# facebookresearch/goliath

Measured on NVIDIA B200. Metric: rendered megapixels/sec (fwd+bwd) RGCA head 300k Gaussians, higher is better.
Workload: dtype f32

## Files before the change

### goliath_b200/csrc/splat_bin_tiles.cu

```cuda
#include <stdlib.h>
#include <string.h>

#include "common.cuh"
#include "splat_record.cuh"

extern "C" int gb_tile_order(int num_tiles, const int32_t* tile_bins, int32_t* order, void* stream);
extern "C" int gb_tile_schedule(int num_tiles, const int32_t* tile_bins, int32_t* sched, void* stream);
GB_API int gb_bin_tiles_pack_ev(int G, const float* xys, const float* depths, const int32_t* radii, const float* conics,
                                const float* colors3, const float* opacity, const float* compensation, int img_h,
                                int img_w, int block_width, int64_t cap, int32_t* tile_bins, int32_t* tile_order,
                                int tile_sched, int32_t* gids_sorted, float* records, int32_t* n_out, int32_t* overflow,
                                void* workspace, void* colors_ready, void* stream);

namespace {

constexpr int kRankBlock = 256;
constexpr int kRadix = 256;
constexpr int kRankPasses = 4;
constexpr int kScatItems = 2;
constexpr int kSortThreads = 512;
constexpr int kCopyBatch = 2;
constexpr int kMaxBitmapBytes = 192 * 1024;
constexpr int kMaxSmemTiles = 20 * 1024;

inline int rank_items(int G) { return G <= 2048 * 192 ? 8 : 16; }

__device__ __forceinline__ int block_exclusive_scan(int v, int* s_warp, int& total) {
  const int lane = threadIdx.x & 31, warp = threadIdx.x >> 5;
  int inc = v;
#pragma unroll
  for (int o = 1; o < 32; o <<= 1) {
    int t = __shfl_up_sync(0xffffffffu, inc, o);
    if (lane >= o) inc += t;
  }
  if (lane == 31) s_warp[warp] = inc;
  __syncthreads();
  if (warp == 0) {
    int w = (lane < (int)(blockDim.x >> 5)) ? s_warp[lane] : 0;
    int winc = w;
#pragma unroll
    for (int o = 1; o < 32; o <<= 1) {
      int t = __shfl_up_sync(0xffffffffu, winc, o);
      if (lane >= o) winc += t;
    }
    s_warp[lane] = winc - w;
    if (lane == 31) s_warp[32] = winc;
  }
  __syncthreads();
  total = s_warp[32];
  const int r = s_warp[warp] + inc - v;
  __syncthreads();
  return r;
}

__device__ __forceinline__ void tile_bbox(float cx, float cy, float radius, int tbx, int tby, int bw, int& x0,
                                          int& y0, int& x1, int& y1) {
  const float fb = (float)bw;
  const float tcx = __fdiv_rn(cx, fb), tcy = __fdiv_rn(cy, fb), tr = __fdiv_rn(radius, fb);
  x0 = min(max(0, __float2int_rz(__fsub_rn(tcx, tr))), tbx);
  x1 = min(max(0, __float2int_rz(__fadd_rn(__fadd_rn(tcx, tr), 1.f))), tbx);
  y0 = min(max(0, __float2int_rz(__fsub_rn(tcy, tr))), tby);
  y1 = min(max(0, __float2int_rz(__fadd_rn(__fadd_rn(tcy, tr), 1.f))), tby);
}

constexpr int kGaussBlock = 1024;
template <int kTileKeys, bool kRank>
__global__ void __launch_bounds__(kGaussBlock) depth_keys_kernel(int G, const float2* __restrict__ xys,
                                                                 const float* __restrict__ depths,
                                                                 const int* __restrict__ radii, int tbx, int tby,
                                                                 int block_width, int smem_tiles,
                                                                 unsigned* __restrict__ keys,
                                                                 unsigned* __restrict__ hist0 ,
                                                                 int* __restrict__ tile_counts,
                                                                 unsigned* __restrict__ key_bits ) {
  constexpr int kItems = kTileKeys / kGaussBlock;
  extern __shared__ int s_cnt[];
  __shared__ unsigned s_hist[kRadix];
  __shared__ unsigned s_or, s_orc, s_max, s_maxc;
  if (threadIdx.x == 0) s_or = s_orc = s_max = s_maxc = 0u;
  if (threadIdx.x < kRadix) s_hist[threadIdx.x] = 0;
  for (int t = threadIdx.x; t < smem_tiles; t += kGaussBlock) s_cnt[t] = 0;
  const int base = blockIdx.x * kTileKeys;
  unsigned k[kItems];
  int r[kItems];
  float2 c[kItems];
#pragma unroll
  for (int j = 0; j < kItems; ++j) {
    const int i = base + j * kGaussBlock + threadIdx.x;
    const bool in = i < G;
    k[j] = in ? __float_as_uint(depths[i]) : 0u;
    r[j] = in ? radii[i] : 0;
    c[j] = in ? xys[i] : make_float2(0.f, 0.f);
  }
  {
    unsigned o = 0u, oc = 0u, mx = 0u, mxc = 0u;
#pragma unroll
    for (int j = 0; j < kItems; ++j)
      if (r[j] > 0) { o |= k[j]; oc |= ~k[j]; mx = max(mx, k[j]); mxc = max(mxc, ~k[j]); }
    o = __reduce_or_sync(0xffffffffu, o);
    oc = __reduce_or_sync(0xffffffffu, oc);
    mx = __reduce_max_sync(0xffffffffu, mx);
    mxc = __reduce_max_sync(0xffffffffu, mxc);
    __syncthreads();
    if ((threadIdx.x & 31) == 0 && (o | oc)) {
      atomicOr(&s_or, o); atomicOr(&s_orc, oc); atomicMax(&s_max, mx); atomicMax(&s_maxc, mxc);
    }
  }
  __syncthreads();
#pragma unroll
  for (int j = 0; j < kItems; ++j) {
    const int i = base + j * kGaussBlock + threadIdx.x;
    if (i >= G) continue;
    if (kRank) {
      keys[i] = k[j];
      atomicAdd(&s_hist[k[j] & 0xffu], 1u);
    }
    if (r[j] > 0) {
      int x0, y0, x1, y1;
      tile_bbox(c[j].x, c[j].y, (float)r[j], tbx, tby, block_width, x0, y0, x1, y1);
      for (int ty = y0; ty < y1; ++ty)
        for (int tx = x0; tx < x1; ++tx) {
          if (smem_tiles) atomicAdd(&s_cnt[ty * tbx + tx], 1);
          else atomicAdd(&tile_counts[ty * tbx + tx], 1);
        }
    }
  }
  __syncthreads();
  if (threadIdx.x == 0 && (s_or | s_orc)) {
    atomicOr(key_bits, s_or); atomicOr(key_bits + 1, s_orc);
    atomicMax(key_bits + 4, s_max); atomicMax(key_bits + 5, s_maxc);
  }
  if (kRank && threadIdx.x < kRadix) hist0[(size_t)blockIdx.x * kRadix + threadIdx.x] = s_hist[threadIdx.x];
  for (int t = threadIdx.x; t < smem_tiles; t += kGaussBlock) {
    const int cnt = s_cnt[t];
    if (cnt) atomicAdd(&tile_counts[t], cnt);
  }
}

template <int kItems>
__global__ void __launch_bounds__(kRankBlock) rank_scatter_kernel(
    int n, const unsigned* __restrict__ keys_in, const int* __restrict__ vals_in ,
    unsigned* __restrict__ keys_out , int* __restrict__ vals_out, int shift, int ctas,
    const unsigned* __restrict__ hist_cur ,
    unsigned* __restrict__ hist_next ,
    int* __restrict__ rank_of ) {
  constexpr int kWarps = kRankBlock / 32;
  constexpr int kTile = kRankBlock * kItems;
  __shared__ unsigned s_whist[kWarps][kRadix];
  __shared__ int s_scan[33];
  const int lane = threadIdx.x & 31, warp = threadIdx.x >> 5;

  const int warp_base = blockIdx.x * kTile + warp * (32 * kItems);
  unsigned k[kItems];
  int v[kItems];
#pragma unroll
  for (int j = 0; j < kItems; ++j) {
    const int i = warp_base + j * 32 + lane;
    k[j] = (i < n) ? keys_in[i] : 0xffffffffu;
    v[j] = (i < n) ? (vals_in ? vals_in[i] : i) : 0;
  }

  __shared__ uint4 s_part[2][4][kRadix / 4];
  {
    const int g = threadIdx.x >> 6, c4 = threadIdx.x & 63;
    const uint4* tab = reinterpret_cast<const uint4*>(hist_cur);
    uint4 tot = make_uint4(0u, 0u, 0u, 0u), bef = make_uint4(0u, 0u, 0u, 0u);
#pragma unroll 8
    for (int b = g; b < ctas; b += 4) {
      const uint4 h = tab[(size_t)b * (kRadix / 4) + c4];
      tot.x += h.x; tot.y += h.y; tot.z += h.z; tot.w += h.w;
      if (b < (int)blockIdx.x) { bef.x += h.x; bef.y += h.y; bef.z += h.z; bef.w += h.w; }
    }
    s_part[0][g][c4] = tot;
    s_part[1][g][c4] = bef;
  }
  __syncthreads();
  unsigned before = 0, total = 0;
  {
    const unsigned* pt = reinterpret_cast<const unsigned*>(&s_part[0][0][0]);
    const unsigned* pb = reinterpret_cast<const unsigned*>(&s_part[1][0][0]);
#pragma unroll
    for (int g = 0; g < 4; ++g) {
      total += pt[g * kRadix + threadIdx.x];
      before += pb[g * kRadix + threadIdx.x];
    }
  }
  const bool copy_only = __syncthreads_or(total == (unsigned)n) != 0;

  if (copy_only) {
#pragma unroll
    for (int j = 0; j < kItems; ++j) {
      const int i = warp_base + j * 32 + lane;
      if (i < n) {
        if (keys_out) keys_out[i] = k[j];
        vals_out[i] = v[j];
        if (hist_next) atomicAdd(&hist_next[(size_t)blockIdx.x * kRadix + ((k[j] >> (shift + 8)) & 0xffu)], 1u);
        if (rank_of) rank_of[v[j]] = i;
      }
    }
    return;
  }
  int unused;
  const unsigned digit_base = (unsigned)block_exclusive_scan((int)total, s_scan, unused);
  const unsigned my_base = digit_base + before;

  for (int d = lane; d < kRadix; d += 32) s_whist[warp][d] = 0;
  __syncwarp();
  unsigned rank[kItems];
#pragma unroll
  for (int j = 0; j < kItems; ++j) {
    const int i = warp_base + j * 32 + lane;
    const bool valid = i < n;
    const unsigned dgt = (k[j] >> shift) & 0xffu;
    const unsigned peers = __match_any_sync(0xffffffffu, valid ? dgt : 0x100u);
    const unsigned lower = peers & ((1u << lane) - 1u);
    unsigned prev = 0;
    if (valid) prev = s_whist[warp][dgt];
    __syncwarp();
    rank[j] = prev + __popc(lower);
    if (valid && lower == 0u) s_whist[warp][dgt] = prev + __popc(peers);
    __syncwarp();
  }
  __syncthreads();
  {
    const int d = threadIdx.x;
    unsigned run = my_base;
#pragma unroll
    for (int w = 0; w < kWarps; ++w) {
      const unsigned c = s_whist[w][d];
      s_whist[w][d] = run;
      run += c;
    }
  }
  __syncthreads();
#pragma unroll
  for (int j = 0; j < kItems; ++j) {
    const int i = warp_base + j * 32 + lane;
    if (i < n) {
      const unsigned dgt = (k[j] >> shift) & 0xffu;
      const unsigned dst = s_whist[warp][dgt] + rank[j];
      if (keys_out) keys_out[dst] = k[j];
      vals_out[dst] = v[j];
      if (hist_next) atomicAdd(&hist_next[(size_t)(dst / kTile) * kRadix + ((k[j] >> (shift + 8)) & 0xffu)], 1u);
      if (rank_of) rank_of[v[j]] = (int)dst;
    }
  }
}


__device__ __forceinline__ void grid_barrier(unsigned* counter, unsigned& target) {
  __syncthreads();
  if (threadIdx.x == 0) {
    target += gridDim.x;
    __threadfence();
    atomicAdd(counter, 1u);
    unsigned seen;
    do {
      asm volatile("ld.acquire.gpu.global.u32 %0, [%1];" : "=r"(seen) : "l"(counter) : "memory");
    } while (seen < target);
    __threadfence();
  }
  __syncthreads();
}

template <int kItems>
__global__ void __launch_bounds__(kRankBlock) rank_sort_coop_kernel(
    int n, int tiles, unsigned* keys_a, unsigned* keys_b, int* vals_a, int* vals_b, unsigned* hist ,
    const unsigned* key_bits, unsigned* barrier , int* __restrict__ rank_to_gid, int* __restrict__ rank_of) {
  constexpr int kWarps = kRankBlock / 32;
  constexpr int kTile = kRankBlock * kItems;
  __shared__ unsigned s_whist[kWarps][kRadix];
  __shared__ int s_scan[33];
  __shared__ uint4 s_part[2][4][kRadix / 4];
  const int lane = threadIdx.x & 31, warp = threadIdx.x >> 5;
  if (key_bits[7] && !key_bits[6]) return;
  const unsigned diff = key_bits[0] & key_bits[1];
  const int bits = diff ? 32 - __clz(diff) : 0;
  const int passes = (bits + 7) >> 3;
  unsigned bar_target = 0;
  const size_t hs = (size_t)tiles * kRadix;

  if (passes == 0) {
    for (int i = blockIdx.x * kRankBlock + threadIdx.x; i < n; i += gridDim.x * kRankBlock) {
      rank_to_gid[i] = i;
      rank_of[i] = i;
    }
    return;
  }
  auto warp_ranks = [&](const unsigned (&k)[kItems], int warp_base, int shift, unsigned (&rank)[kItems]) {
    for (int d = lane; d < kRadix; d += 32) s_whist[warp][d] = 0;
    __syncwarp();
#pragma unroll
    for (int j = 0; j < kItems; ++j) {
      const int i = warp_base + j * 32 + lane;
      const bool valid = i < n;
      const unsigned dgt = (k[j] >> shift) & 0xffu;
      const unsigned peers = __match_any_sync(0xffffffffu, valid ? dgt : 0x100u);
      const unsigned lower = peers & ((1u << lane) - 1u);
      unsigned prev = 0;
      if (valid) prev = s_whist[warp][dgt];
      __syncwarp();
      rank[j] = prev + __popc(lower);
      if (valid && lower == 0u) s_whist[warp][dgt] = prev + __popc(peers);
      __syncwarp();
    }
  };
  for (int p = 0; p < passes; ++p) {
    const bool last = (p == passes - 1);
    const int shift = 8 * p;
    const unsigned* kin = (p & 1) ? keys_b : keys_a;
    unsigned* kout = (p & 1) ? keys_a : keys_b;
    const int* vin = (p == 0) ? nullptr : ((p & 1) ? vals_b : vals_a);
    int* vout = last ? rank_to_gid : ((p & 1) ? vals_a : vals_b);
    unsigned* hist_cur = hist + (size_t)p * hs;
    if (p > 0) {
      for (int tile = blockIdx.x; tile < tiles; tile += gridDim.x) {
        const int warp_base = tile * kTile + warp * (32 * kItems);
        unsigned k[kItems], rank[kItems];
#pragma unroll
        for (int j = 0; j < kItems; ++j) {
          const int i = warp_base + j * 32 + lane;
          k[j] = (i < n) ? __ldcg(kin + i) : 0xffffffffu;
        }
        warp_ranks(k, warp_base, shift, rank);
        __syncthreads();
        {
          unsigned c = 0;
#pragma unroll
          for (int w = 0; w < kWarps; ++w) c += s_whist[w][threadIdx.x];
          hist_cur[(size_t)tile * kRadix + threadIdx.x] = c;
        }
        __syncthreads();
      }
      grid_barrier(barrier, bar_target);
    }
    for (int tile = blockIdx.x; tile < tiles; tile += gridDim.x) {
      const int warp_base = tile * kTile + warp * (32 * kItems);
      unsigned k[kItems];
      int v[kItems];
#pragma unroll
      for (int j = 0; j < kItems; ++j) {
        const int i = warp_base + j * 32 + lane;
        k[j] = (i < n) ? __ldcg(kin + i) : 0xffffffffu;
        v[j] = (i < n) ? (vin ? __ldcg(vin + i) : i) : 0;
      }
      {
        const int g = threadIdx.x >> 6, c4 = threadIdx.x & 63;
        const uint4* tab = reinterpret_cast<const uint4*>(hist_cur);
        uint4 tot = make_uint4(0u, 0u, 0u, 0u), bef = make_uint4(0u, 0u, 0u, 0u);
#pragma unroll 8
        for (int b = g; b < tiles; b += 4) {
          const uint4 h = __ldcg(tab + (size_t)b * (kRadix / 4) + c4);
          tot.x += h.x; tot.y += h.y; tot.z += h.z; tot.w += h.w;
          if (b < tile) { bef.x += h.x; bef.y += h.y; bef.z += h.z; bef.w += h.w; }
        }
        s_part[0][g][c4] = tot;
        s_part[1][g][c4] = bef;
      }
      __syncthreads();
      unsigned before = 0, total = 0;
      {
        const unsigned* pt = reinterpret_cast<const unsigned*>(&s_part[0][0][0]);
        const unsigned* pb = reinterpret_cast<const unsigned*>(&s_part[1][0][0]);
#pragma unroll
        for (int g = 0; g < 4; ++g) {
          total += pt[g * kRadix + threadIdx.x];
          before += pb[g * kRadix + threadIdx.x];
        }
      }
      int unused;
      const unsigned digit_base = (unsigned)block_exclusive_scan((int)total, s_scan, unused);
      const unsigned my_base = digit_base + before;
      unsigned rank[kItems];
      warp_ranks(k, warp_base, shift, rank);
      __syncthreads();
      {
        const int d = threadIdx.x;
        unsigned run = my_base;
#pragma unroll
        for (int w = 0; w < kWarps; ++w) {
          const unsigned c = s_whist[w][d];
          s_whist[w][d] = run;
          run += c;
        }
      }
      __syncthreads();
#pragma unroll
      for (int j = 0; j < kItems; ++j) {
        const int i = warp_base + j * 32 + lane;
        if (i < n) {
          const unsigned dgt = (k[j] >> shift) & 0xffu;
          const unsigned dst = s_whist[warp][dgt] + rank[j];
          if (!last) kout[dst] = k[j];
          else rank_of[v[j]] = (int)dst;
          vout[dst] = v[j];
        }
      }
      __syncthreads();
    }
    if (!last) grid_barrier(barrier, bar_target);
  }
}

constexpr int kBuckets = 2048;
constexpr int kBucketCap = 2048;
constexpr int kBucketThreads = 128;

__device__ __forceinline__ int bucket_of(unsigned key, unsigned kmin, unsigned long long range) {
  return (int)(((unsigned long long)(key - kmin) * (unsigned long long)kBuckets) / range);
}

template <int kTileKeys>
__global__ void __launch_bounds__(kGaussBlock) rank_bucket_count_kernel(int G, const unsigned* __restrict__ keys,
                                                                        const int* __restrict__ radii,
                                                                        const unsigned* __restrict__ key_bits,
                                                                        int* __restrict__ bcount) {
  constexpr int kItems = kTileKeys / kGaussBlock;
  __shared__ int s_cnt[kBuckets];
  for (int t = threadIdx.x; t < kBuckets; t += kGaussBlock) s_cnt[t] = 0;
  const unsigned kmax = key_bits[4], kmin = ~key_bits[5];
  const unsigned long long range = (unsigned long long)(kmax - kmin) + 1ull;
  __syncthreads();
  const int base = blockIdx.x * kTileKeys;
#pragma unroll
  for (int j = 0; j < kItems; ++j) {
    const int i = base + j * kGaussBlock + threadIdx.x;
    if (i < G && radii[i] > 0) atomicAdd(&s_cnt[bucket_of(keys[i], kmin, range)], 1);
  }
  __syncthreads();
  for (int t = threadIdx.x; t < kBuckets; t += kGaussBlock) {
    const int c = s_cnt[t];
    if (c) atomicAdd(&bcount[t], c);
  }
}

__global__ void __launch_bounds__(1024) rank_bucket_scan_kernel(const int* __restrict__ bcount, int* __restrict__ boffset,
                                                                int* __restrict__ bcursor, unsigned* __restrict__ flags) {
  __shared__ int s_warp[33];
  __shared__ int s_max;
  if (threadIdx.x == 0) s_max = 0;
  __syncthreads();
  int carry = 0;
  for (int base = 0; base < kBuckets; base += 1024) {
    const int i = base + threadIdx.x;
    const int v = bcount[i];
    int total;
    const int ex = block_exclusive_scan(v, s_warp, total);
    boffset[i] = carry + ex;
    bcursor[i] = 0;
    atomicMax(&s_max, v);
    carry += total;
  }
  __syncthreads();
  if (threadIdx.x == 0) flags[6] = (s_max > kBucketCap) ? 1u : 0u;
}

template <int kTileKeys>
__global__ void __launch_bounds__(kGaussBlock) rank_bucket_scatter_kernel(int G, const unsigned* __restrict__ keys,
                                                                          const int* __restrict__ radii,
                                                                          const unsigned* __restrict__ key_bits,
                                                                          const int* __restrict__ boffset,
                                                                          int* __restrict__ bcursor,
                                                                          unsigned* __restrict__ pair_keys,
                                                                          int* __restrict__ pair_ids) {
  constexpr int kItems = kTileKeys / kGaussBlock;
  __shared__ int s_cnt[kBuckets];
  __shared__ int s_base[kBuckets];
  if (key_bits[6]) return;
  for (int t = threadIdx.x; t < kBuckets; t += kGaussBlock) s_cnt[t] = 0;
  const unsigned kmax = key_bits[4], kmin = ~key_bits[5];
  const unsigned long long range = (unsigned long long)(kmax - kmin) + 1ull;
  __syncthreads();
  const int base = blockIdx.x * kTileKeys;
  unsigned k[kItems];
  int b[kItems];
#pragma unroll
  for (int j = 0; j < kItems; ++j) {
    const int i = base + j * kGaussBlock + threadIdx.x;
    b[j] = -1;
    if (i < G && radii[i] > 0) {
      k[j] = keys[i];
      b[j] = bucket_of(k[j], kmin, range);
      atomicAdd(&s_cnt[b[j]], 1);
    }
  }
  __syncthreads();
  for (int t = threadIdx.x; t < kBuckets; t += kGaussBlock) {
    const int c = s_cnt[t];
    s_base[t] = c ? boffset[t] + atomicAdd(&bcursor[t], c) : 0;
    s_cnt[t] = 0;
  }
  __syncthreads();
#pragma unroll
  for (int j = 0; j < kItems; ++j) {
    if (b[j] < 0) continue;
    const int pos = s_base[b[j]] + atomicAdd(&s_cnt[b[j]], 1);
    pair_keys[pos] = k[j];
    pair_ids[pos] = base + j * kGaussBlock + threadIdx.x;
  }
}

__global__ void __launch_bounds__(kBucketThreads) rank_bucket_sort_kernel(const int* __restrict__ bcount,
                                                                          const int* __restrict__ boffset,
                                                                          const unsigned* __restrict__ key_bits,
                                                                          const unsigned* __restrict__ pair_keys,
                                                                          const int* __restrict__ pair_ids,
                                                                          int* __restrict__ rank_to_gid, int* __restrict__ rank_of) {
  __shared__ unsigned s_k[kBucketCap];
  __shared__ int s_id[kBucketCap];
  if (key_bits[6]) return;
  const int n = bcount[blockIdx.x], off = boffset[blockIdx.x];
  if (n <= 0) return;
  for (int i = threadIdx.x; i < n; i += kBucketThreads) {
    s_k[i] = pair_keys[off + i];
    s_id[i] = pair_ids[off + i];
  }
  __syncthreads();
  for (int i = threadIdx.x; i < n; i += kBucketThreads) {
    const unsigned ki = s_k[i];
    const int idi = s_id[i];
    int r = 0;
    for (int j = 0; j < n; ++j) {
      const unsigned kj = s_k[j];
      r += (kj < ki || (kj == ki && s_id[j] < idi)) ? 1 : 0;
    }
    rank_to_gid[off + r] = idi;
    rank_of[idi] = off + r;
  }
}

__global__ void __launch_bounds__(1024) tile_scan_kernel(int T, long long cap, const int* __restrict__ counts,
                                                         int2* __restrict__ tile_bins, int* __restrict__ cursor,
                                                         int* __restrict__ n_out, int* __restrict__ overflow) {
  __shared__ int s_warp[33];
  int carry = 0;
  for (int base = 0; base < T; base += blockDim.x) {
    const int i = base + threadIdx.x;
    const int v = (i < T) ? counts[i] : 0;
    int total;
    const int ex = block_exclusive_scan(v, s_warp, total);
    if (i < T) {
      const int s = carry + ex;
      cursor[i] = s;
      const int cs = (int)min((long long)s, cap), ce = (int)min((long long)s + v, cap);
      tile_bins[i] = (ce > cs) ? make_int2(cs, ce) : make_int2(0, 0);
    }
    carry += total;
  }
  if (threadIdx.x == 0) {
    if (n_out) *n_out = carry;
    if (overflow && (long long)carry > cap) *overflow = 1;
  }
}

template <bool kById>
__global__ void __launch_bounds__(kGaussBlock) tile_scatter_kernel(
    int G, const float2* __restrict__ xys, const int* __restrict__ radii, const int* __restrict__ rank_of,
    const float* __restrict__ conics, const float* __restrict__ colors3, const float* __restrict__ depths,
    const float* __restrict__ opacity, const float* __restrict__ comp, int tbx, int tby, int block_width,
    long long cap, int smem_tiles, int* __restrict__ cursor, int* __restrict__ tile_ranks, int* __restrict__ slot_ids,
    float4* __restrict__ rec_by_rank) {
  extern __shared__ int s_cnt[];
  int* s_base = s_cnt + smem_tiles;
  for (int t = threadIdx.x; t < smem_tiles; t += kGaussBlock) s_cnt[t] = 0;
  const int base = blockIdx.x * (kGaussBlock * kScatItems);
  int rk[kScatItems], r[kScatItems];
  float2 c[kScatItems];
#pragma unroll
  for (int j = 0; j < kScatItems; ++j) {
    const int i = base + j * kGaussBlock + threadIdx.x;
    const bool in = i < G;
    r[j] = in ? radii[i] : 0;
    c[j] = in ? xys[i] : make_float2(0.f, 0.f);
    if (kById) rk[j] = in ? __float_as_int(depths[i]) : 0;
    else rk[j] = in ? rank_of[i] : 0;
  }
  __syncthreads();
  unsigned bx[kScatItems], by[kScatItems];
#pragma unroll
  for (int j = 0; j < kScatItems; ++j) {
    const int i = base + j * kGaussBlock + threadIdx.x;
    bx[j] = by[j] = 0u;
    if (r[j] <= 0) continue;
    int x0, y0, x1, y1;
    tile_bbox(c[j].x, c[j].y, (float)r[j], tbx, tby, block_width, x0, y0, x1, y1);
    bx[j] = (unsigned)x0 | ((unsigned)x1 << 16);
    by[j] = (unsigned)y0 | ((unsigned)y1 << 16);
    gb::pack_record_fused(i, xys, conics, colors3, depths, opacity, comp, rec_by_rank + 3 * (size_t)(kById ? i : rk[j]));
    for (int ty = y0; ty < y1; ++ty)
      for (int tx = x0; tx < x1; ++tx) {
        if (smem_tiles) {
          atomicAdd(&s_cnt[ty * tbx + tx], 1);
        } else {
          const int pos = atomicAdd(&cursor[ty * tbx + tx], 1);
          if ((long long)pos < cap) {
            tile_ranks[pos] = rk[j];
            if (kById) slot_ids[pos] = i;
          }
        }
      }
  }
  if (!smem_tiles) return;
  __syncthreads();
  for (int t = threadIdx.x; t < smem_tiles; t += kGaussBlock) {
    const int cnt = s_cnt[t];
    s_base[t] = cnt ? atomicAdd(&cursor[t], cnt) : 0;
    s_cnt[t] = 0;
  }
  __syncthreads();
#pragma unroll
  for (int j = 0; j < kScatItems; ++j) {
    const int x0 = bx[j] & 0xffffu, x1 = bx[j] >> 16, y0 = by[j] & 0xffffu, y1 = by[j] >> 16;
    for (int ty = y0; ty < y1; ++ty)
      for (int tx = x0; tx < x1; ++tx) {
        const int t = ty * tbx + tx;
        const int pos = s_base[t] + atomicAdd(&s_cnt[t], 1);
        if ((long long)pos < cap) {
          tile_ranks[pos] = rk[j];
          if (kById) slot_ids[pos] = base + j * kGaussBlock + threadIdx.x;
        }
      }
  }
}

__global__ void __launch_bounds__(kSortThreads, 3) tile_sort_pack_kernel(
    int words , int chunk , const int* __restrict__ order,
    const int2* __restrict__ tile_bins, const int* __restrict__ tile_ranks, const int* __restrict__ rank_to_gid,
    const float4* __restrict__ rec_by_rank, int* __restrict__ gids_sorted, float4* __restrict__ rec) {
  extern __shared__ unsigned s_bits[];
  __shared__ int s_warp[33];
  const int tile = order ? order[blockIdx.x] : (int)blockIdx.x;
  const int2 range = tile_bins[tile];
  const int n = range.y - range.x;
  if (n <= 0) return;
  for (int w = threadIdx.x; w < words; w += kSortThreads) s_bits[w] = 0u;
  __syncthreads();
  for (int i0 = threadIdx.x; i0 < n; i0 += 4 * kSortThreads) {
    int r[4];
#pragma unroll
    for (int u = 0; u < 4; ++u) {
      const int i = i0 + u * kSortThreads;
      r[u] = (i < n) ? tile_ranks[range.x + i] : -1;
    }
#pragma unroll
    for (int u = 0; u < 4; ++u)
      if (r[u] >= 0) atomicOr(&s_bits[r[u] >> 5], 1u << (r[u] & 31));
  }
  __syncthreads();
  const int w0 = threadIdx.x * chunk, w1 = min(words, w0 + chunk);
  int cnt = 0;
  for (int w = w0; w < w1; ++w) cnt += __popc(s_bits[w]);
  int total;
  int pos = range.x + block_exclusive_scan(cnt, s_warp, total);
  for (int w = w0; w < w1; ++w) {
    unsigned m = s_bits[w];
    while (m) {
      const int b = __ffs(m) - 1;
      m &= m - 1;
      gids_sorted[pos++] = w * 32 + b;
    }
  }
  __syncthreads();
  for (int i0 = threadIdx.x; i0 < n; i0 += kCopyBatch * kSortThreads) {
    int r[kCopyBatch], g[kCopyBatch];
    float4 q[kCopyBatch][3];
#pragma unroll
    for (int u = 0; u < kCopyBatch; ++u) {
      const int i = i0 + u * kSortThreads;
      r[u] = (i < n) ? __ldcg(gids_sorted + (size_t)range.x + i) : -1;
    }
#pragma unroll
    for (int u = 0; u < kCopyBatch; ++u) {
      if (r[u] < 0) continue;
      g[u] = rank_to_gid[r[u]];
      const float4* src = rec_by_rank + 3 * (size_t)r[u];
      q[u][0] = gb::ld_nc_f4(src);
      q[u][1] = gb::ld_nc_f4(src + 1);
      q[u][2] = gb::ld_nc_f4(src + 2);
    }
#pragma unroll
    for (int u = 0; u < kCopyBatch; ++u) {
      if (r[u] < 0) continue;
      const size_t idx = (size_t)range.x + i0 + u * kSortThreads;
      gids_sorted[idx] = g[u];
      rec[3 * idx + 0] = q[u][0];
      rec[3 * idx + 1] = q[u][1];
      rec[3 * idx + 2] = q[u][2];
    }
  }
}

__global__ void __launch_bounds__(kSortThreads, 3) tile_sort_kernel(int words, int chunk, const int* __restrict__ order,
                                                                    const int2* __restrict__ tile_bins,
                                                                    int* __restrict__ tile_ranks) {
  extern __shared__ unsigned s_bits[];
  __shared__ int s_warp[33];
  const int tile = order ? order[blockIdx.x] : (int)blockIdx.x;
  const int2 range = tile_bins[tile];
  const int n = range.y - range.x;
  if (n <= 0) return;
  for (int w = threadIdx.x; w < words; w += kSortThreads) s_bits[w] = 0u;
  __syncthreads();
  for (int i0 = threadIdx.x; i0 < n; i0 += 4 * kSortThreads) {
    int r[4];
#pragma unroll
    for (int u = 0; u < 4; ++u) {
      const int i = i0 + u * kSortThreads;
      r[u] = (i < n) ? tile_ranks[range.x + i] : -1;
    }
#pragma unroll
    for (int u = 0; u < 4; ++u)
      if (r[u] >= 0) atomicOr(&s_bits[r[u] >> 5], 1u << (r[u] & 31));
  }
  __syncthreads();
  const int w0 = threadIdx.x * chunk, w1 = min(words, w0 + chunk);
  int cnt = 0;
  for (int w = w0; w < w1; ++w) cnt += __popc(s_bits[w]);
  int total;
  int pos = range.x + block_exclusive_scan(cnt, s_warp, total);
  for (int w = w0; w < w1; ++w) {
    unsigned m = s_bits[w];
    while (m) {
      const int b = __ffs(m) - 1;
      m &= m - 1;
      tile_ranks[pos++] = w * 32 + b;
    }
  }
}

constexpr int kPairThreads = 512;
constexpr int kPairWarps = kPairThreads / 32;
constexpr int kPairCap = 6144;
constexpr size_t kPairSmem = (size_t)2 * kPairCap * 8 + (size_t)kPairWarps * kRadix * 4;

__device__ __forceinline__ unsigned long long* pair_radix_sort(unsigned long long* a, unsigned long long* b, int n,
                                                               unsigned long long varying, unsigned* s_hist, int* s_warp) {
  const int lane = threadIdx.x & 31, warp = threadIdx.x >> 5;
  const int per = (n + kPairWarps - 1) / kPairWarps;
  const int c0 = min(n, warp * per), c1 = min(n, c0 + per);
  const unsigned lt = (1u << lane) - 1u;
  unsigned* h = s_hist + warp * kRadix;
  for (int shift = 0; shift < 64; shift += 8) {
    if (((varying >> shift) & 0xffull) == 0ull) continue;
    for (int d = lane; d < kRadix; d += 32) h[d] = 0u;
    __syncwarp();
    for (int i = c0 + lane; i < c1; i += 32) atomicAdd(&h[(unsigned)(a[i] >> shift) & 0xffu], 1u);
    __syncthreads();
    {
      const int d = threadIdx.x;
      unsigned tot = 0u;
      if (d < kRadix)
        for (int w = 0; w < kPairWarps; ++w) tot += s_hist[w * kRadix + d];
      int unused;
      unsigned run = (unsigned)block_exclusive_scan((int)tot, s_warp, unused);
      if (d < kRadix)
        for (int w = 0; w < kPairWarps; ++w) {
          const unsigned c = s_hist[w * kRadix + d];
          s_hist[w * kRadix + d] = run;
          run += c;
        }
    }
    __syncthreads();
    for (int i0 = c0; i0 < c1; i0 += 32) {
      const int i = i0 + lane;
      const bool valid = i < c1;
      const unsigned long long v = valid ? a[i] : 0ull;
      const unsigned dg = valid ? ((unsigned)(v >> shift) & 0xffu) : 0x100u;
      const unsigned peers = __match_any_sync(0xffffffffu, dg);
      const unsigned lower = peers & lt;
      const unsigned at = valid ? h[dg] : 0u;
      __syncwarp();
      if (valid) {
        b[at + __popc(lower)] = v;
        if (lower == 0u) h[dg] = at + __popc(peers);
      }
      __syncwarp();
    }
    __syncthreads();
    unsigned long long* t = a;
    a = b;
    b = t;
  }
  return a;
}

constexpr int kMaxRun = 32;
__device__ __forceinline__ void pair_sort_tile(unsigned long long* a, unsigned long long* b, int2 range,
                                               unsigned kmin, const unsigned* __restrict__ tile_keys,
                                               int* __restrict__ gids_sorted, unsigned* s_hist, int* s_warp,
                                               unsigned long long* s_or_and) {
  const int n = range.y - range.x;
  unsigned long long o = 0ull, an = ~0ull;
  for (int i0 = threadIdx.x; i0 < n; i0 += 4 * kPairThreads) {
    unsigned k[4];
    int g[4];
#pragma unroll
    for (int u = 0; u < 4; ++u) {
      const int i = i0 + u * kPairThreads;
      k[u] = (i < n) ? tile_keys[range.x + i] : kmin;
      g[u] = (i < n) ? gids_sorted[range.x + i] : 0;
    }
#pragma unroll
    for (int u = 0; u < 4; ++u) {
      const int i = i0 + u * kPairThreads;
      if (i < n) {
        const unsigned long long c = ((unsigned long long)(k[u] - kmin) << 32) | (unsigned)g[u];
        a[i] = c;
        o |= c;
        an &= c;
      }
    }
  }
  const unsigned olo = __reduce_or_sync(0xffffffffu, (unsigned)o), ohi = __reduce_or_sync(0xffffffffu, (unsigned)(o >> 32));
  const unsigned alo = __reduce_and_sync(0xffffffffu, (unsigned)an),
                 ahi = __reduce_and_sync(0xffffffffu, (unsigned)(an >> 32));
  if ((threadIdx.x & 31) == 0) {
    atomicOr(&s_or_and[0], ((unsigned long long)ohi << 32) | olo);
    atomicAnd(&s_or_and[1], ((unsigned long long)ahi << 32) | alo);
  }
  __syncthreads();
  const unsigned long long varying = s_or_and[0] & ~s_or_and[1];
  unsigned long long* res = pair_radix_sort(a, b, n, varying & 0xffffffff00000000ull, s_hist, s_warp);
  bool long_run = false;
  for (int i = threadIdx.x; i < n; i += kPairThreads) {
    const unsigned key = (unsigned)(res[i] >> 32);
    if (i > 0 && (unsigned)(res[i - 1] >> 32) == key) continue;
    int e = i + 1;
    while (e < n && e - i <= kMaxRun && (unsigned)(res[e] >> 32) == key) ++e;
    if (e - i > kMaxRun) {
      long_run = true;
    } else {
      for (int j = i + 1; j < e; ++j) {
        const unsigned long long v = res[j];
        int p = j - 1;
        while (p >= i && res[p] > v) {
          res[p + 1] = res[p];
          --p;
        }
        res[p + 1] = v;
      }
    }
  }
  if (__syncthreads_or(long_run)) res = pair_radix_sort(res, res == a ? b : a, n, varying, s_hist, s_warp);
  for (int i = threadIdx.x; i < n; i += kPairThreads) gids_sorted[range.x + i] = (int)(unsigned)res[i];
}

__global__ void __launch_bounds__(kPairThreads, 2) tile_pair_sort_kernel(
    const int* __restrict__ order, const int2* __restrict__ tile_bins,
    const unsigned* __restrict__ key_bits , const unsigned* __restrict__ tile_keys,
    int* __restrict__ gids_sorted, float* __restrict__ records ) {
  extern __shared__ unsigned long long s_pairs[];
  __shared__ int s_warp[33];
  __shared__ unsigned long long s_or_and[2];
  const int tile = order ? order[blockIdx.x] : (int)blockIdx.x;
  const int2 range = tile_bins[tile];
  const int n = range.y - range.x;
  if (n <= 1) return;
  if (threadIdx.x == 0) {
    s_or_and[0] = 0ull;
    s_or_and[1] = ~0ull;
  }
  __syncthreads();
  const unsigned kmin = ~key_bits[5];
  unsigned* s_hist = reinterpret_cast<unsigned*>(s_pairs + 2 * kPairCap);
  if (n <= kPairCap) {
    pair_sort_tile(s_pairs, s_pairs + kPairCap, range, kmin, tile_keys, gids_sorted, s_hist, s_warp, s_or_and);
  } else {
    unsigned long long* a = reinterpret_cast<unsigned long long*>(records + 12 * (size_t)range.x);
    pair_sort_tile(a, a + n, range, kmin, tile_keys, gids_sorted, s_hist, s_warp, s_or_and);
  }
}

__global__ void __launch_bounds__(256) rec_colors_kernel(int G, const int* __restrict__ radii,
                                                         const int* __restrict__ rank_of,
                                                         const float* __restrict__ colors3,
                                                         const float* __restrict__ depths, float4* __restrict__ rec_by_rank) {
  const int g = blockIdx.x * blockDim.x + threadIdx.x;
  if (g >= G || radii[g] <= 0) return;
  const size_t at = rank_of ? (size_t)rank_of[g] : (size_t)g;
  rec_by_rank[3 * at + 2] = make_float4(colors3[3 * (size_t)g], colors3[3 * (size_t)g + 1], colors3[3 * (size_t)g + 2],
                                        depths[g]);
}

__global__ void __launch_bounds__(256) gather_records_kernel(long long cap, const int* __restrict__ n_dev,
                                                             const int* ranks_sorted, const int* __restrict__ rank_to_gid,
                                                             const float4* __restrict__ rec_by_rank, int* gids_sorted,
                                                             float4* __restrict__ rec) {
  const long long n = min((long long)*n_dev, cap);
  const long long j = (long long)blockIdx.x * blockDim.x + threadIdx.x;
  if (j >= 3 * n) return;
  const long long i = j / 3;
  const int part = (int)(j - 3 * i);
  const int r = ranks_sorted[i];
  rec[j] = gb::ld_nc_f4(rec_by_rank + 3 * (size_t)r + part);
  if (rank_to_gid && part == 0) gids_sorted[i] = rank_to_gid[r];
}

struct Layout {
  size_t counts, hist, buckets, sync, zero_bytes, cursor, keys_a, keys_b, vals_a, vals_b, rank_to_gid, rank_of, rec_by_rank,
      tile_ranks, total;
};
inline size_t align256(size_t b) { return (b + 255) & ~(size_t)255; }
inline Layout make_layout(int G, int T, int64_t cap) {
  const int g1 = G > 0 ? G : 1;
  const size_t ctas = (size_t)gb::cdiv(g1, kRankBlock * rank_items(g1));
  const size_t g4 = align256((size_t)g1 * 4);
  Layout l;
  size_t o = 0;
  l.counts = o; o += align256((size_t)T * 4);
  l.hist = o;   o += align256(ctas * kRadix * 4 * kRankPasses);
  l.buckets = o; o += align256((size_t)3 * 2048 * 4);
  l.sync = o;   o += 256;
  l.zero_bytes = o;
  l.cursor = o; o += align256((size_t)T * 4);
  l.keys_a = o; o += g4;
  l.keys_b = o; o += g4;
  l.vals_a = o; o += g4;
  l.vals_b = o; o += g4;
  l.rank_to_gid = o; o += g4;
  l.rank_of = o; o += g4;
  l.rec_by_rank = o; o += align256((size_t)g1 * 48);
  l.tile_ranks = o; o += align256((size_t)(cap > 0 ? cap : 1) * 4);
  l.total = o;
  return l;
}

int g_tile_sort_mode = -1;
int tile_sort_mode() {
  if (g_tile_sort_mode < 0) {
    const char* e = getenv("GOLIATH_B200_TILESORT");
    g_tile_sort_mode = (e && strcmp(e, "fused") == 0) ? 1 : 0;
  }
  return g_tile_sort_mode;
}
int g_bin_sort_mode = -1;
int bin_sort_mode() {
  if (g_bin_sort_mode < 0) {
    const char* e = getenv("GOLIATH_B200_BINSORT");
    g_bin_sort_mode = (e && strcmp(e, "rank") == 0) ? 1 : 0;
  }
  return g_bin_sort_mode;
}
int g_rank_sort_mode = -1;
int rank_sort_mode() {
  if (g_rank_sort_mode < 0) {
    const char* e = getenv("GOLIATH_B200_RANKSORT");
    g_rank_sort_mode = !e ? 0 : strcmp(e, "passes") == 0 ? 1 : strcmp(e, "buckets") == 0 ? 2 : 0;
  }
  return g_rank_sort_mode;
}
int sm_count() {
  static int n[64] = {};
  int dev = 0;
  if (cudaGetDevice(&dev) != cudaSuccess || dev < 0 || dev >= 64) return gb::kNumSMs;
  if (!n[dev]) {
    int v = 0;
    if (cudaDeviceGetAttribute(&v, cudaDevAttrMultiProcessorCount, dev) != cudaSuccess || v < 1) v = gb::kNumSMs;
    n[dev] = v;
  }
  return n[dev];
}

template <int kItems>
int launch_rank_sort(int G, int ctas, const float* xys, const float* depths, const int32_t* radii, int tbx, int tby,
                     int block_width, int smem_tiles, unsigned* keys_a, unsigned* keys_b, int* vals_a, int* vals_b,
                     unsigned* hist, int* counts, int* buckets, unsigned* sync, int* rank_to_gid, int* rank_of, cudaStream_t s) {
  const size_t hs = (size_t)ctas * kRadix;
  depth_keys_kernel<kRankBlock * kItems, true><<<ctas, kGaussBlock, (size_t)smem_tiles * 4, s>>>(
      G, (const float2*)xys, depths, radii, tbx, tby, block_width, smem_tiles, keys_a, hist, counts, sync);
  const int mode = rank_sort_mode();
  if (mode == 2) {
    int* bcount = buckets;
    int* boffset = bcount + kBuckets;
    int* bcursor = boffset + kBuckets;
    rank_bucket_count_kernel<kRankBlock * kItems><<<ctas, kGaussBlock, 0, s>>>(G, keys_a, radii, sync, bcount);
    rank_bucket_scan_kernel<<<1, 1024, 0, s>>>(bcount, boffset, bcursor, sync);
    rank_bucket_scatter_kernel<kRankBlock * kItems><<<ctas, kGaussBlock, 0, s>>>(G, keys_a, radii, sync, boffset, bcursor, keys_b,
                                                                               vals_b);
    rank_bucket_sort_kernel<<<kBuckets, kBucketThreads, 0, s>>>(bcount, boffset, sync, keys_b, vals_b, rank_to_gid, rank_of);
    gb::count_launches(4);
  }
  if (mode == 0 || mode == 2) {
    int n = G, tiles = ctas;
    const unsigned* key_bits = sync;
    unsigned* barrier = sync + 2;
    void* args[] = {&n, &tiles, &keys_a, &keys_b, &vals_a, &vals_b, &hist, &key_bits, &barrier, &rank_to_gid, &rank_of};
    const int grid = ctas < sm_count() ? ctas : sm_count();
    if (mode == 2) GB_CUDA(cudaMemsetAsync(sync + 7, 0xff, 4, s));
    GB_CUDA(cudaLaunchCooperativeKernel((const void*)rank_sort_coop_kernel<kItems>, dim3(grid), dim3(kRankBlock), args, 0, s));
    gb::count_launches(2);
    return 0;
  }
  rank_scatter_kernel<kItems><<<ctas, kRankBlock, 0, s>>>(G, keys_a, nullptr, keys_b, vals_b, 0, ctas, hist, hist + hs,
                                                          nullptr);
  rank_scatter_kernel<kItems><<<ctas, kRankBlock, 0, s>>>(G, keys_b, vals_b, keys_a, vals_a, 8, ctas, hist + hs,
                                                          hist + 2 * hs, nullptr);
  rank_scatter_kernel<kItems><<<ctas, kRankBlock, 0, s>>>(G, keys_a, vals_a, keys_b, vals_b, 16, ctas, hist + 2 * hs,
                                                          hist + 3 * hs, nullptr);
  rank_scatter_kernel<kItems><<<ctas, kRankBlock, 0, s>>>(G, keys_b, vals_b, nullptr, rank_to_gid, 24, ctas, hist + 3 * hs,
                                                          nullptr, rank_of);
  gb::count_launches(5);
  return 0;
}

template <typename K>
int opt_in_smem(K kernel, bool* done) {
  int dev = 0;
  GB_CUDA(cudaGetDevice(&dev));
  if (dev < 0 || dev >= 64 || !done[dev]) {
    GB_CUDA(cudaFuncSetAttribute(kernel, cudaFuncAttributeMaxDynamicSharedMemorySize, kMaxBitmapBytes));
    if (dev >= 0 && dev < 64) done[dev] = true;
  }
  return 0;
}

}

GB_API int gb_get_bin_sort_mode(void) { return bin_sort_mode(); }
GB_API void gb_set_bin_sort_mode(int mode) { g_bin_sort_mode = mode ? 1 : 0; }
GB_API int gb_get_tile_sort_mode(void) { return tile_sort_mode(); }
GB_API void gb_set_tile_sort_mode(int mode) { g_tile_sort_mode = mode ? 1 : 0; }
GB_API int gb_get_rank_sort_mode(void) { return rank_sort_mode(); }
GB_API void gb_set_rank_sort_mode(int mode) { g_rank_sort_mode = mode < 0 ? 0 : (mode > 2 ? 2 : mode); }

GB_API int gb_bin_tiles_supported(int G) { return G >= 1 && ((size_t)gb::cdiv(G, 32) * 4 <= (size_t)kMaxBitmapBytes); }

GB_API size_t gb_bin_tiles_workspace_bytes(int G, int num_tiles, int64_t cap) {
  return make_layout(G, num_tiles, cap).total;
}

GB_API int gb_bin_tiles_pack(int G, const float* xys, const float* depths, const int32_t* radii, const float* conics,
                             const float* colors3, const float* opacity, const float* compensation, int img_h,
                             int img_w, int block_width, int64_t cap, int32_t* tile_bins, int32_t* tile_order,
                             int tile_sched, int32_t* gids_sorted, float* records, int32_t* n_out, int32_t* overflow,
                             void* workspace, void* stream) {
  return gb_bin_tiles_pack_ev(G, xys, depths, radii, conics, colors3, opacity, compensation, img_h, img_w, block_width, cap,
                              tile_bins, tile_order, tile_sched, gids_sorted, records, n_out, overflow, workspace, nullptr,
                              stream);
}

static int bin_tiles_impl(int G, const float* xys, const float* depths, const int32_t* radii, const float* conics,
                          const float* colors3, const float* opacity, const float* compensation, int img_h, int img_w,
                          int block_width, int64_t cap, int32_t* tile_bins, int32_t* tile_order, int tile_sched,
                          int32_t* gids_sorted, float* records, int32_t* n_out, int32_t* overflow, void* workspace,
                          void* colors_ready, void* stream, int32_t* ext_ranks, float* ext_rec, int32_t* ext_r2g);

GB_API int gb_bin_tiles_pack_ev(int G, const float* xys, const float* depths, const int32_t* radii, const float* conics,
                                const float* colors3, const float* opacity, const float* compensation, int img_h,
                                int img_w, int block_width, int64_t cap, int32_t* tile_bins, int32_t* tile_order,
                                int tile_sched, int32_t* gids_sorted, float* records, int32_t* n_out, int32_t* overflow,
                                void* workspace, void* colors_ready, void* stream) {
  return bin_tiles_impl(G, xys, depths, radii, conics, colors3, opacity, compensation, img_h, img_w, block_width, cap,
                        tile_bins, tile_order, tile_sched, gids_sorted, records, n_out, overflow, workspace, colors_ready,
                        stream, nullptr, nullptr, nullptr);
}

GB_API int gb_bin_tiles_ranked(int G, const float* xys, const float* depths, const int32_t* radii, const float* conics,
                               const float* colors3, const float* opacity, const float* compensation, int img_h,
                               int img_w, int block_width, int64_t cap, int32_t* tile_bins, int32_t* tile_order,
                               int tile_sched, int32_t* ranks_sorted, float* rec_by_rank, int32_t* rank_to_gid,
                               int32_t* n_out, int32_t* overflow, void* workspace, void* colors_ready, void* stream) {
  if (!ranks_sorted || !rec_by_rank || !rank_to_gid) return (int)cudaErrorInvalidValue;
  return bin_tiles_impl(G, xys, depths, radii, conics, colors3, opacity, compensation, img_h, img_w, block_width, cap,
                        tile_bins, tile_order, tile_sched, nullptr, nullptr, n_out, overflow, workspace, colors_ready, stream,
                        ranks_sorted, rec_by_rank, rank_to_gid);
}

static int bin_tiles_impl(int G, const float* xys, const float* depths, const int32_t* radii, const float* conics,
                          const float* colors3, const float* opacity, const float* compensation, int img_h, int img_w,
                          int block_width, int64_t cap, int32_t* tile_bins, int32_t* tile_order, int tile_sched,
                          int32_t* gids_sorted, float* records, int32_t* n_out, int32_t* overflow, void* workspace,
                          void* colors_ready, void* stream, int32_t* ext_ranks, float* ext_rec, int32_t* ext_r2g) {
  if (!gb_bin_tiles_supported(G) || block_width < 1 || cap < 0) return (int)cudaErrorInvalidValue;
  cudaStream_t s = (cudaStream_t)stream;
  const int tbx = gb::cdiv(img_w, block_width), tby = gb::cdiv(img_h, block_width);
  const int T = tbx * tby;
  if (T < 1 || tbx > 65535 || tby > 65535) return (int)cudaErrorInvalidValue;
  const Layout l = make_layout(G, T, cap);
  char* ws = (char*)workspace;
  int* counts = (int*)(ws + l.counts);
  unsigned* hist = (unsigned*)(ws + l.hist);
  int* cursor = (int*)(ws + l.cursor);
  unsigned* keys_a = (unsigned*)(ws + l.keys_a);
  unsigned* keys_b = (unsigned*)(ws + l.keys_b);
  int* vals_a = (int*)(ws + l.vals_a);
  int* vals_b = (int*)(ws + l.vals_b);
  const bool ranked = ext_ranks != nullptr;
  int* rank_to_gid = ranked ? ext_r2g : (int*)(ws + l.rank_to_gid);
  unsigned* sync = (unsigned*)(ws + l.sync);
  int* rank_of = (int*)(ws + l.rank_of);
  float4* rec_by_rank = ranked ? (float4*)ext_rec : (float4*)(ws + l.rec_by_rank);
  int* tile_ranks = ranked ? ext_ranks : (int*)(ws + l.tile_ranks);
  const int items = rank_items(G);
  const int ctas = gb::cdiv(G, kRankBlock * items);
  const int smem_tiles = (T <= kMaxSmemTiles) ? T : 0;
  const bool by_id = !ranked && bin_sort_mode() == 0;
  static bool s_opt_k8[64] = {}, s_opt_k16[64] = {}, s_opt_scat[64] = {}, s_opt_sort[64] = {}, s_opt_sort2[64] = {};
  static bool s_opt_k8i[64] = {}, s_opt_k16i[64] = {}, s_opt_scati[64] = {}, s_opt_pair[64] = {};
  if ((size_t)smem_tiles * 8 > 40 * 1024) {
    int e = by_id ? ((items == 8) ? opt_in_smem(depth_keys_kernel<kRankBlock * 8, false>, s_opt_k8i)
                                  : opt_in_smem(depth_keys_kernel<kRankBlock * 16, false>, s_opt_k16i))
                  : ((items == 8) ? opt_in_smem(depth_keys_kernel<kRankBlock * 8, true>, s_opt_k8)
                                  : opt_in_smem(depth_keys_kernel<kRankBlock * 16, true>, s_opt_k16));
    if (e) return e;
    e = by_id ? opt_in_smem(tile_scatter_kernel<true>, s_opt_scati) : opt_in_smem(tile_scatter_kernel<false>, s_opt_scat);
    if (e) return e;
  }

  GB_CUDA(cudaMemsetAsync(ws, 0, l.zero_bytes, s));
  if (by_id) {
    if (items == 8)
      depth_keys_kernel<kRankBlock * 8, false><<<ctas, kGaussBlock, (size_t)smem_tiles * 4, s>>>(
          G, (const float2*)xys, depths, radii, tbx, tby, block_width, smem_tiles, nullptr, nullptr, counts, sync);
    else
      depth_keys_kernel<kRankBlock * 16, false><<<ctas, kGaussBlock, (size_t)smem_tiles * 4, s>>>(
          G, (const float2*)xys, depths, radii, tbx, tby, block_width, smem_tiles, nullptr, nullptr, counts, sync);
    gb::count_launches(1);
  } else {
    const int es = (items == 8)
                       ? launch_rank_sort<8>(G, ctas, xys, depths, radii, tbx, tby, block_width, smem_tiles, keys_a, keys_b,
                                             vals_a, vals_b, hist, counts, (int*)(ws + l.buckets), sync, rank_to_gid, rank_of, s)
                       : launch_rank_sort<16>(G, ctas, xys, depths, radii, tbx, tby, block_width, smem_tiles, keys_a, keys_b,
                                              vals_a, vals_b, hist, counts, (int*)(ws + l.buckets), sync, rank_to_gid, rank_of, s);
    if (es) return es;
  }
  int* n_total = n_out ? n_out : (int*)(sync + 3);
  tile_scan_kernel<<<1, 1024, 0, s>>>(T, (long long)cap, counts, (int2*)tile_bins, cursor, n_total, overflow);
  gb::count_launches(1);
  GB_CHECK_LAUNCH();
  const int e = tile_sched ? gb_tile_schedule(T, tile_bins, tile_order, stream)
                           : gb_tile_order(T, tile_bins, tile_order, stream);
  if (e) return e;
  const bool split = by_id || ranked || tile_sort_mode() == 0;
  const bool late = split && colors_ready;
  if (!late && colors_ready) GB_CUDA(cudaStreamWaitEvent(s, (cudaEvent_t)colors_ready, 0));
  const int scat_ctas = gb::cdiv(G, kGaussBlock * kScatItems);
  if (by_id) {
    tile_scatter_kernel<true><<<scat_ctas, kGaussBlock, (size_t)smem_tiles * 8, s>>>(
        G, (const float2*)xys, radii, nullptr, conics, late ? nullptr : colors3, depths, opacity, compensation, tbx, tby,
        block_width, (long long)cap, smem_tiles, cursor, tile_ranks, gids_sorted, rec_by_rank);
    if (cap > 0) {
      const int e2 = opt_in_smem(tile_pair_sort_kernel, s_opt_pair);
      if (e2) return e2;
      tile_pair_sort_kernel<<<T, kPairThreads, kPairSmem, s>>>(tile_order, (const int2*)tile_bins, sync,
                                                               (const unsigned*)tile_ranks, gids_sorted, records);
    }
    if (late) {
      GB_CUDA(cudaStreamWaitEvent(s, (cudaEvent_t)colors_ready, 0));
      rec_colors_kernel<<<gb::cdiv(G, 256), 256, 0, s>>>(G, radii, nullptr, colors3, depths, rec_by_rank);
      gb::count_launches(1);
    }
    if (cap > 0)
      gather_records_kernel<<<(unsigned)gb::cdiv64(3 * cap, 256), 256, 0, s>>>((long long)cap, n_total, gids_sorted, nullptr,
                                                                               rec_by_rank, gids_sorted, (float4*)records);
    gb::count_launches(3);
    GB_CHECK_LAUNCH();
    return 0;
  }
  tile_scatter_kernel<false><<<scat_ctas, kGaussBlock, (size_t)smem_tiles * 8, s>>>(
      G, (const float2*)xys, radii, rank_of, conics, late ? nullptr : colors3, depths, opacity, compensation, tbx, tby,
      block_width, (long long)cap, smem_tiles, cursor, tile_ranks, nullptr, rec_by_rank);
  const int words = gb::cdiv(G, 32);
  const int chunk = gb::cdiv(words, kSortThreads) | 1;
  const size_t smem = (size_t)words * 4;
  if (split) {
    if (smem > 40 * 1024) {
      const int e2 = opt_in_smem(tile_sort_kernel, s_opt_sort2);
      if (e2) return e2;
    }
    tile_sort_kernel<<<T, kSortThreads, smem, s>>>(words, chunk, tile_order, (const int2*)tile_bins, tile_ranks);
    if (late) {
      GB_CUDA(cudaStreamWaitEvent(s, (cudaEvent_t)colors_ready, 0));
      rec_colors_kernel<<<gb::cdiv(G, 256), 256, 0, s>>>(G, radii, rank_of, colors3, depths, rec_by_rank);
      gb::count_launches(1);
    }
    if (cap > 0 && !ranked)
      gather_records_kernel<<<(unsigned)gb::cdiv64(3 * cap, 256), 256, 0, s>>>((long long)cap, n_total, tile_ranks, rank_to_gid,
                                                                             rec_by_rank, gids_sorted, (float4*)records);
    gb::count_launches(3);
    GB_CHECK_LAUNCH();
    return 0;
  }
  if (smem > 40 * 1024) {
    const int e2 = opt_in_smem(tile_sort_pack_kernel, s_opt_sort);
    if (e2) return e2;
  }
  tile_sort_pack_kernel<<<T, kSortThreads, smem, s>>>(words, chunk, tile_order, (const int2*)tile_bins, tile_ranks,
                                                      rank_to_gid, rec_by_rank, gids_sorted, (float4*)records);
  gb::count_launches(2);
  GB_CHECK_LAUNCH();
  return 0;
}
```

Before: 1808.

## Bucket-sort tile pairs and fuse record gather into tile pair sort kernel

Replaces the per-tile 64-bit radix sort with a depth-range bucket sort that uses 4096 buckets plus in-bucket rank counting. It falls back to radix sort when the estimated quadratic work is too high. The separate gather_records kernel is folded into the pair-sort kernel, which reads sorted gids straight from shared memory. The colors kernel now runs before the sort to meet the dependency, which removes a launch and a global pass over gids. The risks are a skewed depth distribution causing quadratic in-bucket ranking, and the colors wait now blocking the sort.

```diff
diff --git a/goliath_b200/csrc/splat_bin_tiles.cu b/goliath_b200/csrc/splat_bin_tiles.cu
--- a/goliath_b200/csrc/splat_bin_tiles.cu
+++ b/goliath_b200/csrc/splat_bin_tiles.cu
@@ -731,7 +731,14 @@
 constexpr int kPairThreads = 512;
 constexpr int kPairWarps = kPairThreads / 32;
 constexpr int kPairCap = 6144;
+constexpr int kBucketBitsTile = 12;
+constexpr int kTileBuckets = 1 << kBucketBitsTile;
+constexpr int kBucketWork = 32;
+constexpr int kPairLoad = 8;
+constexpr int kPackBatch = 8;
 constexpr size_t kPairSmem = (size_t)2 * kPairCap * 8 + (size_t)kPairWarps * kRadix * 4;
+static_assert(kTileBuckets == kPairWarps * kRadix, "bucket counters share the warp histograms' space");
+static_assert(kTileBuckets == 8 * kPairThreads, "each thread scans 8 bucket counters");
 
 __device__ __forceinline__ unsigned long long* pair_radix_sort(unsigned long long* a, unsigned long long* b, int n,
                                                                unsigned long long varying, unsigned* s_hist, int* s_warp) {
@@ -784,90 +791,163 @@
   return a;
 }
 
-constexpr int kMaxRun = 32;
-__device__ __forceinline__ void pair_sort_tile(unsigned long long* a, unsigned long long* b, int2 range,
-                                               unsigned kmin, const unsigned* __restrict__ tile_keys,
-                                               int* __restrict__ gids_sorted, unsigned* s_hist, int* s_warp,
-                                               unsigned long long* s_or_and) {
+struct PairTileSmem {
+  unsigned long long or_and[2];
+  unsigned kmin, kmax;
+  unsigned long long work;
+};
+
+__device__ __forceinline__ unsigned long long* pair_sort_tile(unsigned long long* a, unsigned long long* b, int2 range,
+                                                              unsigned kmin, const unsigned* __restrict__ tile_keys,
+                                                              int* __restrict__ gids_sorted, unsigned* s_cnt, int* s_warp,
+                                                              PairTileSmem& sm) {
   const int n = range.y - range.x;
+  if (threadIdx.x == 0) {
+    sm.or_and[0] = 0ull;
+    sm.or_and[1] = ~0ull;
+    sm.kmin = ~0u;
+    sm.kmax = 0u;
+    sm.work = 0ull;
+  }
+  for (int d = threadIdx.x; d < kTileBuckets; d += kPairThreads) s_cnt[d] = 0u;
+  __syncthreads();
   unsigned long long o = 0ull, an = ~0ull;
-  for (int i0 = threadIdx.x; i0 < n; i0 += 4 * kPairThreads) {
-    unsigned k[4];
-    int g[4];
-#pragma unroll
-    for (int u = 0; u < 4; ++u) {
+  unsigned lo = ~0u, hi = 0u;
+  for (int i0 = threadIdx.x; i0 < n; i0 += kPairLoad * kPairThreads) {
+    unsigned k[kPairLoad];
+    int g[kPairLoad];
+#pragma unroll
+    for (int u = 0; u < kPairLoad; ++u) {
       const int i = i0 + u * kPairThreads;
       k[u] = (i < n) ? tile_keys[range.x + i] : kmin;
       g[u] = (i < n) ? gids_sorted[range.x + i] : 0;
     }
 #pragma unroll
-    for (int u = 0; u < 4; ++u) {
+    for (int u = 0; u < kPairLoad; ++u) {
       const int i = i0 + u * kPairThreads;
       if (i < n) {
-        const unsigned long long c = ((unsigned long long)(k[u] - kmin) << 32) | (unsigned)g[u];
+        const unsigned kk = k[u] - kmin;
+        const unsigned long long c = ((unsigned long long)kk << 32) | (unsigned)g[u];
         a[i] = c;
         o |= c;
         an &= c;
+        lo = min(lo, kk);
+        hi = max(hi, kk);
       }
     }
   }
-  const unsigned olo = __reduce_or_sync(0xffffffffu, (unsigned)o), ohi = __reduce_or_sync(0xffffffffu, (unsigned)(o >> 32));
-  const unsigned alo = __reduce_and_sync(0xffffffffu, (unsigned)an),
-                 ahi = __reduce_and_sync(0xffffffffu, (unsigned)(an >> 32));
-  if ((threadIdx.x & 31) == 0) {
-    atomicOr(&s_or_and[0], ((unsigned long long)ohi << 32) | olo);
-    atomicAnd(&s_or_and[1], ((unsigned long long)ahi << 32) | alo);
-  }
-  __syncthreads();
-  const unsigned long long varying = s_or_and[0] & ~s_or_and[1];
-  unsigned long long* res = pair_radix_sort(a, b, n, varying & 0xffffffff00000000ull, s_hist, s_warp);
-  bool long_run = false;
-  for (int i = threadIdx.x; i < n; i += kPairThreads) {
-    const unsigned key = (unsigned)(res[i] >> 32);
-    if (i > 0 && (unsigned)(res[i - 1] >> 32) == key) continue;
-    int e = i + 1;
-    while (e < n && e - i <= kMaxRun && (unsigned)(res[e] >> 32) == key) ++e;
-    if (e - i > kMaxRun) {
-      long_run = true;
-    } else {
-      for (int j = i + 1; j < e; ++j) {
-        const unsigned long long v = res[j];
-        int p = j - 1;
-        while (p >= i && res[p] > v) {
-          res[p + 1] = res[p];
-          --p;
-        }
-        res[p + 1] = v;
-      }
-    }
-  }
-  if (__syncthreads_or(long_run)) res = pair_radix_sort(res, res == a ? b : a, n, varying, s_hist, s_warp);
+  {
+    const unsigned olo = __reduce_or_sync(0xffffffffu, (unsigned)o), ohi = __reduce_or_sync(0xffffffffu, (unsigned)(o >> 32));
+    const unsigned alo = __reduce_and_sync(0xffffffffu, (unsigned)an),
+                   ahi = __reduce_and_sync(0xffffffffu, (unsigned)(an >> 32));
+    lo = __reduce_min_sync(0xffffffffu, lo);
+    hi = __reduce_max_sync(0xffffffffu, hi);
+    if ((threadIdx.x & 31) == 0) {
+      atomicOr(&sm.or_and[0], ((unsigned long long)ohi << 32) | olo);
+      atomicAnd(&sm.or_and[1], ((unsigned long long)ahi << 32) | alo);
+      atomicMin(&sm.kmin, lo);
+      atomicMax(&sm.kmax, hi);
+    }
+  }
+  __syncthreads();
+  const unsigned tmin = sm.kmin, span = sm.kmax - tmin;
+  const int shift = max(0, (32 - __clz(span)) - kBucketBitsTile);
+  auto bucket = [&](unsigned long long c) { return (int)(((unsigned)(c >> 32) - tmin) >> shift); };
+  for (int i = threadIdx.x; i < n; i += kPairThreads) atomicAdd(&s_cnt[bucket(a[i])], 1u);
+  __syncthreads();
+  {
+    uint4* c4 = reinterpret_cast<uint4*>(s_cnt) + 2 * threadIdx.x;
+    uint4 p = c4[0], q = c4[1];
+    const unsigned sum = p.x + p.y + p.z + p.w + q.x + q.y + q.z + q.w;
+    auto sq = [](unsigned v) { return (unsigned long long)v * v; };
+    const unsigned long long w = sq(p.x) + sq(p.y) + sq(p.z) + sq(p.w) + sq(q.x) + sq(q.y) + sq(q.z) + sq(q.w);
+    if (w) atomicAdd(&sm.work, w);
+    int unused;
+    unsigned run = (unsigned)block_exclusive_scan((int)sum, s_warp, unused);
+    unsigned t;
+    t = p.x; p.x = run; run += t;
+    t = p.y; p.y = run; run += t;
+    t = p.z; p.z = run; run += t;
+    t = p.w; p.w = run; run += t;
+    t = q.x; q.x = run; run += t;
+    t = q.y; q.y = run; run += t;
+    t = q.z; q.z = run; run += t;
+    q.w = run;
+    c4[0] = p;
+    c4[1] = q;
+  }
+  __syncthreads();
+  unsigned long long* res;
+  if (sm.work > (unsigned long long)kBucketWork * (unsigned long long)n) {
+    res = pair_radix_sort(a, b, n, sm.or_and[0] & ~sm.or_and[1], s_cnt, s_warp);
+  } else {
+#pragma unroll 4
+    for (int i = threadIdx.x; i < n; i += kPairThreads) {
+      const unsigned long long c = a[i];
+      b[atomicAdd(&s_cnt[bucket(c)], 1u)] = c;
+    }
+    __syncthreads();
+#pragma unroll 2
+    for (int p = threadIdx.x; p < n; p += kPairThreads) {
+      const unsigned long long c = b[p];
+      const int k = bucket(c);
+      const int s = k ? (int)s_cnt[k - 1] : 0, e = (int)s_cnt[k];
+      int r = 0;
+      for (int j = s; j < e; ++j) r += (b[j] < c) ? 1 : 0;
+      a[s + r] = c;
+    }
+    __syncthreads();
+    res = a;
+  }
   for (int i = threadIdx.x; i < n; i += kPairThreads) gids_sorted[range.x + i] = (int)(unsigned)res[i];
+  return res;
 }
 
 __global__ void __launch_bounds__(kPairThreads, 2) tile_pair_sort_kernel(
     const int* __restrict__ order, const int2* __restrict__ tile_bins,
     const unsigned* __restrict__ key_bits , const unsigned* __restrict__ tile_keys,
-    int* __restrict__ gids_sorted, float* __restrict__ records ) {
+    const float4* __restrict__ rec_by_id, int* __restrict__ gids_sorted, float4* __restrict__ records) {
   extern __shared__ unsigned long long s_pairs[];
   __shared__ int s_warp[33];
-  __shared__ unsigned long long s_or_and[2];
+  __shared__ PairTileSmem sm;
   const int tile = order ? order[blockIdx.x] : (int)blockIdx.x;
   const int2 range = tile_bins[tile];
   const int n = range.y - range.x;
-  if (n <= 1) return;
-  if (threadIdx.x == 0) {
-    s_or_and[0] = 0ull;
-    s_or_and[1] = ~0ull;
-  }
-  __syncthreads();
+  if (n <= 0) return;
+  float4* dst = records + 3 * (size_t)range.x;
+  if (n == 1) {
+    if (threadIdx.x < 3) dst[threadIdx.x] = gb::ld_nc_f4(rec_by_id + 3 * (size_t)gids_sorted[range.x] + threadIdx.x);
+    return;
+  }
   const unsigned kmin = ~key_bits[5];
-  unsigned* s_hist = reinterpret_cast<unsigned*>(s_pairs + 2 * kPairCap);
-  if (n <= kPairCap) {
-    pair_sort_tile(s_pairs, s_pairs + kPairCap, range, kmin, tile_keys, gids_sorted, s_hist, s_warp, s_or_and);
+  unsigned* s_cnt = reinterpret_cast<unsigned*>(s_pairs + 2 * kPairCap);
+  const bool in_smem = n <= kPairCap;
+  const unsigned long long* res;
+  if (in_smem) {
+    res = pair_sort_tile(s_pairs, s_pairs + kPairCap, range, kmin, tile_keys, gids_sorted, s_cnt, s_warp, sm);
   } else {
-    unsigned long long* a = reinterpret_cast<unsigned long long*>(records + 12 * (size_t)range.x);
-    pair_sort_tile(a, a + n, range, kmin, tile_keys, gids_sorted, s_hist, s_warp, s_or_and);
+    unsigned long long* a = reinterpret_cast<unsigned long long*>(dst);
+    pair_sort_tile(a, a + n, range, kmin, tile_keys, gids_sorted, s_cnt, s_warp, sm);
+    __syncthreads();
+    res = nullptr;
+  }
+  const int parts = 3 * n;
+  for (int j0 = threadIdx.x; j0 < parts; j0 += kPackBatch * kPairThreads) {
+    float4 q[kPackBatch];
+#pragma unroll
+    for (int u = 0; u < kPackBatch; ++u) {
+      const int j = j0 + u * kPairThreads;
+      if (j < parts) {
+        const int i = j / 3;
+        const int g = in_smem ? (int)(unsigned)res[i] : __ldcg(gids_sorted + range.x + i);
+        q[u] = gb::ld_nc_f4(rec_by_id + 3 * (size_t)g + (j - 3 * i));
+      }
+    }
+#pragma unroll
+    for (int u = 0; u < kPackBatch; ++u) {
+      const int j = j0 + u * kPairThreads;
+      if (j < parts) dst[j] = q[u];
+    }
   }
 }
 
@@ -1139,21 +1219,19 @@
     tile_scatter_kernel<true><<<scat_ctas, kGaussBlock, (size_t)smem_tiles * 8, s>>>(
         G, (const float2*)xys, radii, nullptr, conics, late ? nullptr : colors3, depths, opacity, compensation, tbx, tby,
         block_width, (long long)cap, smem_tiles, cursor, tile_ranks, gids_sorted, rec_by_rank);
+    if (late) {
+      GB_CUDA(cudaStreamWaitEvent(s, (cudaEvent_t)colors_ready, 0));
+      rec_colors_kernel<<<gb::cdiv(G, 256), 256, 0, s>>>(G, radii, nullptr, colors3, depths, rec_by_rank);
+      gb::count_launches(1);
+    }
     if (cap > 0) {
       const int e2 = opt_in_smem(tile_pair_sort_kernel, s_opt_pair);
       if (e2) return e2;
       tile_pair_sort_kernel<<<T, kPairThreads, kPairSmem, s>>>(tile_order, (const int2*)tile_bins, sync,
-                                                               (const unsigned*)tile_ranks, gids_sorted, records);
-    }
-    if (late) {
-      GB_CUDA(cudaStreamWaitEvent(s, (cudaEvent_t)colors_ready, 0));
-      rec_colors_kernel<<<gb::cdiv(G, 256), 256, 0, s>>>(G, radii, nullptr, colors3, depths, rec_by_rank);
-      gb::count_launches(1);
-    }
-    if (cap > 0)
-      gather_records_kernel<<<(unsigned)gb::cdiv64(3 * cap, 256), 256, 0, s>>>((long long)cap, n_total, gids_sorted, nullptr,
-                                                                               rec_by_rank, gids_sorted, (float4*)records);
-    gb::count_launches(3);
+                                                               (const unsigned*)tile_ranks, rec_by_rank, gids_sorted,
+                                                               (float4*)records);
+    }
+    gb::count_launches(2);
     GB_CHECK_LAUNCH();
     return 0;
   }
```

Result: slower. 1767 (median of 6 runs) (-2.3%).
